# NVlabs/CenterPose

Hardware: AMD Instinct MI355X
Metric: images/sec at 512x512 DLA-34 (backbone + heat-map decode + post-process + PnP) (higher is better)
Workload: dtype f32 via split-f16 (f16x3) MFMA, f32 accumulate

## Files before the change

centerpose_amd/csrc/pw16.hip:

```cpp
#include "igemm16_common.h"

namespace {

constexpr int DA = 6;
constexpr int DB = 3;

template <int NT>
__global__ __launch_bounds__(256, 2) void pw16_kernel(const ConvParams p, const int tiles_m, const int tiles_n) {
    typedef Frag<32> F;
    typedef F::acc_t acc_t;
    const int lane = threadIdx.x & 63;
    const int wid = __builtin_amdgcn_readfirstlane(threadIdx.x >> 6);
    const int tile = tile_of_block(tiles_m, tiles_n);
    const int tn = tile % tiles_n, tm = tile / tiles_n;
    const int M = p.B * p.Ho * p.Wo;
    float afwd, ainv;
    conv_in_scale(p, &afwd, &ainv);

    const int row = tm * 128 + wid * 32 + (lane & 31), half = lane >> 5;
    const int n0 = p.src_c[0] >> 4, n1 = p.nsrc > 1 ? p.src_c[1] >> 4 : 0, n2 = p.nsrc > 2 ? p.src_c[2] >> 4 : 0;
    const __amdgpu_buffer_rsrc_t r0 = make_rsrc(p.src[0], (unsigned)M * (unsigned)p.src_c[0] * 4u);
    const __amdgpu_buffer_rsrc_t r1 = make_rsrc(p.nsrc > 1 ? p.src[1] : p.src[0], p.nsrc > 1 ? (unsigned)M * (unsigned)p.src_c[1] * 4u : 0u);
    const __amdgpu_buffer_rsrc_t r2 = make_rsrc(p.nsrc > 2 ? p.src[2] : p.src[0], p.nsrc > 2 ? (unsigned)M * (unsigned)p.src_c[2] * 4u : 0u);
    const __amdgpu_buffer_rsrc_t r3 = make_rsrc(p.nsrc > 3 ? p.src[3] : p.src[0], p.nsrc > 3 ? (unsigned)M * (unsigned)p.src_c[3] * 4u : 0u);
    const bool live = row < M;
    const unsigned v0 = live ? (unsigned)(row * p.src_c[0] + half * 8) * 4u : OOB;
    const unsigned v1 = live && p.nsrc > 1 ? (unsigned)(row * p.src_c[1] + half * 8) * 4u : OOB;
    const unsigned v2 = live && p.nsrc > 2 ? (unsigned)(row * p.src_c[2] + half * 8) * 4u : OOB;
    const unsigned v3 = live && p.nsrc > 3 ? (unsigned)(row * p.src_c[3] + half * 8) * 4u : OOB;
    const int G = p.Kpad16 >> 4;

    const unsigned w_bytes = (unsigned)((size_t)p.CoutPad * p.Kpad16 * 2);
    const __amdgpu_buffer_rsrc_t r_wh = make_rsrc(p.w16f_hi, w_bytes), r_wl = make_rsrc(p.w16f_lo, w_bytes);
    unsigned bd_off[NT];
#pragma unroll
    for (int j = 0; j < NT; ++j) bd_off[j] = (unsigned)((((tn * NT + j) * G) * 64 + lane) * 16);

    u32x4 ra[DA][2];
    u32x4 rbh[DB][NT], rbl[DB][NT];
    auto issue_a = [&](int set, int g) {
        if (g >= G) return;
        int kk = g;
        if (kk < n0) {
            ra[set][0] = __builtin_amdgcn_raw_buffer_load_b128(r0, (int)v0, kk * 64, 0);
            ra[set][1] = __builtin_amdgcn_raw_buffer_load_b128(r0, (int)v0, kk * 64 + 16, 0);
            return;
        }
        kk -= n0;
        if (kk < n1) {
            ra[set][0] = __builtin_amdgcn_raw_buffer_load_b128(r1, (int)v1, kk * 64, 0);
            ra[set][1] = __builtin_amdgcn_raw_buffer_load_b128(r1, (int)v1, kk * 64 + 16, 0);
            return;
        }
        kk -= n1;
        if (kk < n2) {
            ra[set][0] = __builtin_amdgcn_raw_buffer_load_b128(r2, (int)v2, kk * 64, 0);
            ra[set][1] = __builtin_amdgcn_raw_buffer_load_b128(r2, (int)v2, kk * 64 + 16, 0);
            return;
        }
        kk -= n2;
        ra[set][0] = __builtin_amdgcn_raw_buffer_load_b128(r3, (int)v3, kk * 64, 0);
        ra[set][1] = __builtin_amdgcn_raw_buffer_load_b128(r3, (int)v3, kk * 64 + 16, 0);
    };
    auto issue_b = [&](int set, int g) {
        if (g >= G) return;
#pragma unroll
        for (int j = 0; j < NT; ++j) {
            rbh[set][j] = __builtin_amdgcn_raw_buffer_load_b128(r_wh, (int)bd_off[j], g * 1024, 0);
            rbl[set][j] = __builtin_amdgcn_raw_buffer_load_b128(r_wl, (int)bd_off[j], g * 1024, 0);
        }
    };

    acc_t acc[1][NT];
#pragma unroll
    for (int j = 0; j < NT; ++j)
#pragma unroll
        for (int r = 0; r < F::NACC; ++r) acc[0][j][r] = 0.f;

#pragma unroll
    for (int u = 0; u < DB; ++u) issue_b(u, u);
#pragma unroll
    for (int u = 0; u < DA; ++u) issue_a(u, u);

    for (int g0 = 0; g0 < G; g0 += DA) {
#pragma unroll
        for (int u = 0; u < DA; ++u) {
            const int g = g0 + u;
            if (g < G) {
                const u32x4 x0 = ra[u][0], x1 = ra[u][1];
                const Split2 s0 = split2(__uint_as_float(x0.x) * afwd, __uint_as_float(x0.y) * afwd);
                const Split2 s1 = split2(__uint_as_float(x0.z) * afwd, __uint_as_float(x0.w) * afwd);
                const Split2 s2 = split2(__uint_as_float(x1.x) * afwd, __uint_as_float(x1.y) * afwd);
                const Split2 s3 = split2(__uint_as_float(x1.z) * afwd, __uint_as_float(x1.w) * afwd);
                const u32x4 hv = {s0.hi, s1.hi, s2.hi, s3.hi}, lv = {s0.lo, s1.lo, s2.lo, s3.lo};
                const h8 ah = *reinterpret_cast<const h8*>(&hv), al = *reinterpret_cast<const h8*>(&lv);
                issue_a(u, g + DA);
                __builtin_amdgcn_sched_barrier(0);
                constexpr int DBm = DB;
                const int sb = u % DBm;
#pragma unroll
                for (int j = 0; j < NT; ++j)
                    acc[0][j] = __builtin_amdgcn_mfma_f32_32x32x16_f16(al, *reinterpret_cast<const h8*>(&rbh[sb][j]), acc[0][j], 0, 0, 0);
#pragma unroll
                for (int j = 0; j < NT; ++j)
                    acc[0][j] = __builtin_amdgcn_mfma_f32_32x32x16_f16(ah, *reinterpret_cast<const h8*>(&rbl[sb][j]), acc[0][j], 0, 0, 0);
#pragma unroll
                for (int j = 0; j < NT; ++j)
                    acc[0][j] = __builtin_amdgcn_mfma_f32_32x32x16_f16(ah, *reinterpret_cast<const h8*>(&rbh[sb][j]), acc[0][j], 0, 0, 0);
                __builtin_amdgcn_sched_barrier(0);
                issue_b(sb, g + DB);
                __builtin_amdgcn_sched_barrier(0);
            }
        }
    }
    igemm_epilogue<32, 1, NT, 4, 1, false>(p, acc, tm, tn, wid, 0, lane, ainv);
}

constexpr int PA = 3;
constexpr int PW_PITCH = 80;
constexpr int PW_PLANE = 32 * PW_PITCH;

template <int NT>
__device__ __forceinline__ void pw16s_pool_epilogue(const ConvParams& p, f32x16 (&acc)[1][NT], const int tn, const int lane, const float ainv,
                                                    const bool live, const int pair_row, const int blk) {
    const int lcol = lane & 31, h = lane >> 5, W = p.Wo;
    const bool relu = p.act == CP_ACT_RELU;
    float amax = 0.f;
    if (live) {
        const size_t base = (size_t)(2 * pair_row) * W + 16 * blk;
        const __amdgpu_buffer_rsrc_t ro = make_rsrc(p.out + base * p.ldo, (unsigned)((W + 16) * p.ldo) * 4u);
        const __amdgpu_buffer_rsrc_t rp = make_rsrc(p.pool_out + ((size_t)pair_row * (W >> 1) + 8 * blk) * p.ldo, (unsigned)(8 * p.ldo) * 4u);
#pragma unroll
        for (int j = 0; j < NT; ++j) {
            const int n = tn * (32 * NT) + j * 32 + lcol;
            const float sc = (p.scale ? p.scale[n] : 1.f) * ainv;
            const float sh = p.shift ? p.shift[n] : 0.f;
            const bool n_ok = n < p.Cout;
            float v[16];
#pragma unroll
            for (int r = 0; r < 16; ++r) v[r] = acc[0][j][r] * sc + sh;
            if (relu) {
#pragma unroll
                for (int r = 0; r < 16; ++r) v[r] = fmaxf(v[r], 0.f);
            }
#pragma unroll
            for (int r = 0; r < 16; ++r) amax = fmaxf(amax, fabsf(v[r]));
            const unsigned vo = n_ok ? (unsigned)(4 * h * p.ldo + n) * 4u : 0x80000000u;
#pragma unroll
            for (int r = 0; r < 16; ++r)
                __builtin_amdgcn_raw_buffer_store_b32(__float_as_uint(v[r]), ro, (int)vo, ((r >> 3) * W + (r & 3) + 8 * ((r >> 2) & 1)) * p.ldo * 4, 0);
            const unsigned vp = n_ok ? (unsigned)(2 * h * p.ldo + n) * 4u : 0x80000000u;
#pragma unroll
            for (int q = 0; q < 4; ++q) {
                const int r = 2 * q;
                const float mx = fmaxf(fmaxf(v[r], v[r + 1]), fmaxf(v[r + 8], v[r + 9]));
                __builtin_amdgcn_raw_buffer_store_b32(__float_as_uint(mx), rp, (int)vp, ((q & 1) + 4 * (q >> 1)) * p.ldo * 4, 0);
            }
        }
    }
    if (p.out_amax) cp_amax_commit(p.out_amax, amax);
}

template <int NT, bool POOL>
__global__ __launch_bounds__(256, NT == 2 ? 3 : 2) void pw16s_kernel(const ConvParams p, const int tiles_m, const int tiles_n) {
    typedef Frag<32> F;
    typedef F::acc_t acc_t;
    __shared__ __attribute__((aligned(16))) unsigned char stage_s[4][2 * PW_PLANE];
    const int lane = threadIdx.x & 63;
    const int wid = __builtin_amdgcn_readfirstlane(threadIdx.x >> 6);
    const int tile = tile_of_block(tiles_m, tiles_n);
    const int tn = tile % tiles_n, tm = tile / tiles_n;
    const int M = p.B * p.Ho * p.Wo;
    float afwd, ainv;
    conv_in_scale(p, &afwd, &ainv);
    unsigned char* st_hi = stage_s[wid];
    unsigned char* st_lo = st_hi + PW_PLANE;

    const int grp = 4 * tm + wid, wblk = POOL ? p.Wo >> 4 : 1;
    const int pair_row = POOL ? grp / wblk : 0, blk = POOL ? grp - pair_row * wblk : 0;
    const bool live = !POOL || pair_row < p.B * (p.Ho >> 1);
    const int c4 = lane & 7, row0 = POOL ? 2 * pair_row * p.Wo + 16 * blk + (lane >> 3) : tm * 128 + wid * 32 + (lane >> 3);
    const int n0 = p.src_c[0] >> 5, n1 = p.nsrc > 1 ? p.src_c[1] >> 5 : 0, n2 = p.nsrc > 2 ? p.src_c[2] >> 5 : 0;
    const __amdgpu_buffer_rsrc_t r0 = make_rsrc(p.src[0], (unsigned)M * (unsigned)p.src_c[0] * 4u);
    const __amdgpu_buffer_rsrc_t r1 = make_rsrc(p.nsrc > 1 ? p.src[1] : p.src[0], p.nsrc > 1 ? (unsigned)M * (unsigned)p.src_c[1] * 4u : 0u);
    const __amdgpu_buffer_rsrc_t r2 = make_rsrc(p.nsrc > 2 ? p.src[2] : p.src[0], p.nsrc > 2 ? (unsigned)M * (unsigned)p.src_c[2] * 4u : 0u);
    const __amdgpu_buffer_rsrc_t r3 = make_rsrc(p.nsrc > 3 ? p.src[3] : p.src[0], p.nsrc > 3 ? (unsigned)M * (unsigned)p.src_c[3] * 4u : 0u);
    const int GC = live ? p.Kpad16 >> 5 : 0;

    const unsigned w_bytes = (unsigned)((size_t)p.CoutPad * p.Kpad16 * 2);
    const __amdgpu_buffer_rsrc_t r_wh = make_rsrc(p.w16f_hi, w_bytes), r_wl = make_rsrc(p.w16f_lo, w_bytes);
    const int G = p.Kpad16 >> 4;
    unsigned bd_off[NT];
#pragma unroll
    for (int j = 0; j < NT; ++j) bd_off[j] = (unsigned)((((tn * NT + j) * G) * 64 + lane) * 16);

    u32x4 ra[PA][4];
    u32x4 rbh[DB][NT], rbl[DB][NT];
    auto load4 = [&](u32x4 (&dst)[4], const __amdgpu_buffer_rsrc_t r, const int cs, const int kk) {
        const unsigned v = (unsigned)row0 * (unsigned)(cs * 4) + (unsigned)(c4 * 16);
#pragma unroll
        for (int i = 0; i < 4; ++i)
            dst[i] = __builtin_amdgcn_raw_buffer_load_b128(r, (int)v, kk * 128 + (POOL ? (i >> 1) * p.Wo + (i & 1) * 8 : i * 8) * cs * 4, 0);
    };
    auto issue_a = [&](int set, int c) {
        if (c >= GC) return;
        int kk = c;
        if (kk < n0) { load4(ra[set], r0, p.src_c[0], kk); return; }
        kk -= n0;
        if (kk < n1) { load4(ra[set], r1, p.src_c[1], kk); return; }
        kk -= n1;
        if (kk < n2) { load4(ra[set], r2, p.src_c[2], kk); return; }
        kk -= n2;
        load4(ra[set], r3, p.src_c[3], kk);
    };
    auto issue_b = [&](int set, int g) {
        if (g >= G) return;
#pragma unroll
        for (int j = 0; j < NT; ++j) {
            rbh[set][j] = __builtin_amdgcn_raw_buffer_load_b128(r_wh, (int)bd_off[j], g * 1024, 0);
            rbl[set][j] = __builtin_amdgcn_raw_buffer_load_b128(r_wl, (int)bd_off[j], g * 1024, 0);
        }
    };

    acc_t acc[1][NT];
#pragma unroll
    for (int j = 0; j < NT; ++j)
#pragma unroll
        for (int r = 0; r < F::NACC; ++r) acc[0][j][r] = 0.f;

#pragma unroll
    for (int u = 0; u < DB; ++u) issue_b(u, u);
#pragma unroll
    for (int u = 0; u < PA; ++u) issue_a(u, u);

    const int wr_off = (lane >> 3) * PW_PITCH + c4 * 8;
    const int rd_off = (lane & 31) * PW_PITCH + (lane >> 5) * 16;
    static_assert((2 * PA) % DB == 0, "the B register set of a K step must be a compile-time index");
    for (int c0 = 0; c0 < GC; c0 += PA) {
#pragma unroll
        for (int u = 0; u < PA; ++u) {
            const int c = c0 + u;
            if (c < GC) {
#pragma unroll
                for (int i = 0; i < 4; ++i) {
                    const u32x4 x = ra[u][i];
                    const Split2 s0 = split2(__uint_as_float(x.x) * afwd, __uint_as_float(x.y) * afwd);
                    const Split2 s1 = split2(__uint_as_float(x.z) * afwd, __uint_as_float(x.w) * afwd);
                    *reinterpret_cast<u32x2*>(st_hi + wr_off + 8 * i * PW_PITCH) = u32x2{s0.hi, s1.hi};
                    *reinterpret_cast<u32x2*>(st_lo + wr_off + 8 * i * PW_PITCH) = u32x2{s0.lo, s1.lo};
                }
                issue_a(u, c + PA);
                __builtin_amdgcn_wave_barrier();
                h8 ah[2], al[2];
#pragma unroll
                for (int h = 0; h < 2; ++h) {
                    ah[h] = *reinterpret_cast<const h8*>(st_hi + rd_off + 32 * h);
                    al[h] = *reinterpret_cast<const h8*>(st_lo + rd_off + 32 * h);
                }
                __builtin_amdgcn_wave_barrier();
#pragma unroll
                for (int h = 0; h < 2; ++h) {
                    const int g = 2 * c + h;
                    const int sb = (2 * u + h) % DB;
                    __builtin_amdgcn_sched_barrier(0);
#pragma unroll
                    for (int j = 0; j < NT; ++j)
                        acc[0][j] = __builtin_amdgcn_mfma_f32_32x32x16_f16(al[h], *reinterpret_cast<const h8*>(&rbh[sb][j]), acc[0][j], 0, 0, 0);
#pragma unroll
                    for (int j = 0; j < NT; ++j)
                        acc[0][j] = __builtin_amdgcn_mfma_f32_32x32x16_f16(ah[h], *reinterpret_cast<const h8*>(&rbl[sb][j]), acc[0][j], 0, 0, 0);
#pragma unroll
                    for (int j = 0; j < NT; ++j)
                        acc[0][j] = __builtin_amdgcn_mfma_f32_32x32x16_f16(ah[h], *reinterpret_cast<const h8*>(&rbh[sb][j]), acc[0][j], 0, 0, 0);
                    __builtin_amdgcn_sched_barrier(0);
                    issue_b(sb, g + DB);
                    __builtin_amdgcn_sched_barrier(0);
                }
            }
        }
    }
    if (POOL) pw16s_pool_epilogue<NT>(p, acc, tn, lane, ainv, live, pair_row, blk);
    else igemm_epilogue<32, 1, NT, 4, 1, false>(p, acc, tm, tn, wid, 0, lane, ainv);
}

template <int NT>
int launch_pw16s(const ConvParams& p, hipStream_t stream) {
    const int M = p.B * p.Ho * p.Wo;
    const int tiles_m = (M + 127) / 128, tiles_n = p.CoutPad / (32 * NT);
    if (p.pool_out) hipLaunchKernelGGL((pw16s_kernel<NT, true>), dim3(tiles_m * tiles_n), dim3(256), 0, stream, p, tiles_m, tiles_n);
    else hipLaunchKernelGGL((pw16s_kernel<NT, false>), dim3(tiles_m * tiles_n), dim3(256), 0, stream, p, tiles_m, tiles_n);
    return hipGetLastError() == hipSuccess ? CP_OK : CP_ERR_LAUNCH;
}

template <int NT>
int launch_pw16(const ConvParams& p, hipStream_t stream) {
    const int M = p.B * p.Ho * p.Wo;
    const int tiles_m = (M + 127) / 128, tiles_n = p.CoutPad / (32 * NT);
    hipLaunchKernelGGL((pw16_kernel<NT>), dim3(tiles_m * tiles_n), dim3(256), 0, stream, p, tiles_m, tiles_n);
    return hipGetLastError() == hipSuccess ? CP_OK : CP_ERR_LAUNCH;
}

}

static_assert(DA % DB == 0, "the B register set of a K step must be a compile-time index");

bool cp_pw16_supported(const ConvParams& p) {
    if (!p.w16f_hi || !p.w16f_lo || p.KH != 1 || p.KW != 1 || p.stride != 1 || p.pad != 0 || p.H != p.Ho || p.W != p.Wo)
        return false;
    if (p.offmask || p.gn_in_a || p.gn_in_d || p.gn_in_mr || p.gn_stats || p.splitk > 1 || p.nsrc < 1 || p.nsrc > 4)
        return false;
    if (p.CoutPad % 64 != 0 || p.Kpad16 != p.Cin || p.Cin % 32 != 0) return false;
    int c = 0;
    const size_t M = (size_t)p.B * p.Ho * p.Wo;
    for (int s = 0; s < p.nsrc; ++s) {
        if (p.src_c[s] % 32 != 0 || M * p.src_c[s] * 4 >= (size_t)0xf0000000u) return false;
        c += p.src_c[s];
    }
    return c == p.Cin && (size_t)p.CoutPad * p.Kpad16 * 2 < (size_t)0x7fffffff && M * p.ldo * 4 < (size_t)0xf0000000u;
}

bool cp_pw16_pool_supported(const ConvParams& p) {
    if (!cp_pw16_supported(p) || (p.dbg & CP_SEL_PW16_FRAG_A)) return false;
    if (p.res || p.gn_stats || p.store != CP_STORE_NHWC || p.coff != 0 || (p.act != CP_ACT_NONE && p.act != CP_ACT_RELU)) return false;
    return p.Ho % 2 == 0 && p.Wo % 16 == 0;
}

int cp_launch_pw16(const ConvParams& p, hipStream_t stream) {
    if (!cp_pw16_supported(p) || (p.pool_out && !cp_pw16_pool_supported(p))) return CP_ERR_INVALID;
    if (!(p.dbg & CP_SEL_PW16_FRAG_A)) return p.CoutPad % 128 == 0 ? launch_pw16s<4>(p, stream) : launch_pw16s<2>(p, stream);
    return p.CoutPad % 128 == 0 ? launch_pw16<4>(p, stream) : launch_pw16<2>(p, stream);
}
```

Measured before the change: 4771.

## Stage pointwise-conv weights through LDS shared across waves in pw16 kernel

New measurement: 4791, median of 6. No clear change (+0.4%).

```diff
diff --git a/centerpose_amd/csrc/pw16.hip b/centerpose_amd/csrc/pw16.hip
--- a/centerpose_amd/csrc/pw16.hip
+++ b/centerpose_amd/csrc/pw16.hip
@@ -283,6 +283,170 @@
     else igemm_epilogue<32, 1, NT, 4, 1, false>(p, acc, tm, tn, wid, 0, lane, ainv);
 }
 
+template <class T>
+__device__ __forceinline__ T pw16w_pick(const bool a, const bool b, const bool c, const T x0, const T x1, const T x2, const T x3) {
+    const T t2 = c ? T(x2) : T(x3), t1 = b ? T(x1) : t2;
+    return a ? T(x0) : t1;
+}
+
+template <int NT, bool POOL>
+__global__ __launch_bounds__(256, NT == 2 ? 3 : 2) void pw16w_kernel(const ConvParams p, const int tiles_m, const int tiles_n) {
+    typedef Frag<32> F;
+    typedef F::acc_t acc_t;
+    constexpr int BLK = 4 * NT * 1024;
+    __shared__ __attribute__((aligned(16))) unsigned char stage_s[4][2 * PW_PLANE];
+    __shared__ __attribute__((aligned(16))) unsigned char wts_s[2][BLK];
+    const int lane = threadIdx.x & 63;
+    const int wid = __builtin_amdgcn_readfirstlane(threadIdx.x >> 6);
+    const int tile = tile_of_block(tiles_m, tiles_n);
+    const int tn = tile % tiles_n, tm = tile / tiles_n;
+    const int M = p.B * p.Ho * p.Wo;
+    float afwd, ainv;
+    conv_in_scale(p, &afwd, &ainv);
+    unsigned char* st_hi = stage_s[wid];
+    unsigned char* st_lo = st_hi + PW_PLANE;
+
+    const int grp = 4 * tm + wid, wblk = POOL ? p.Wo >> 4 : 1;
+    const int pair_row = POOL ? grp / wblk : 0, blk = POOL ? grp - pair_row * wblk : 0;
+    const bool live = !POOL || pair_row < p.B * (p.Ho >> 1);
+    const int c4 = lane & 7, row0 = POOL ? 2 * pair_row * p.Wo + 16 * blk + (lane >> 3) : tm * 128 + wid * 32 + (lane >> 3);
+    auto opaque = [](const float* q) __attribute__((always_inline)) {
+        const unsigned long long v = (unsigned long long)q;
+        const unsigned lo = __builtin_amdgcn_readfirstlane((unsigned)v), hi = __builtin_amdgcn_readfirstlane((unsigned)(v >> 32));
+        return (const float*)(((unsigned long long)hi << 32) | lo);
+    };
+    const float* const q0 = opaque(p.src[0]);
+    const float* const q1 = opaque(p.src[1]);
+    const float* const q2 = opaque(p.src[2]);
+    const float* const q3 = opaque(p.src[3]);
+    const int cs0 = __builtin_amdgcn_readfirstlane(p.src_c[0]), cs1 = __builtin_amdgcn_readfirstlane(p.nsrc > 1 ? p.src_c[1] : 0);
+    const int cs2 = __builtin_amdgcn_readfirstlane(p.nsrc > 2 ? p.src_c[2] : 0), cs3 = __builtin_amdgcn_readfirstlane(p.nsrc > 3 ? p.src_c[3] : 0);
+    const int e0 = cs0 >> 5, e1 = e0 + (cs1 >> 5), e2 = e1 + (cs2 >> 5);
+    const int GC = p.Kpad16 >> 5;
+
+    const unsigned w_bytes = (unsigned)((size_t)p.CoutPad * p.Kpad16 * 2);
+    const void* const w_hi = p.w16f_hi;
+    const void* const w_lo = p.w16f_lo;
+    const void* const w_ptr = (wid & 1) ? w_lo : w_hi;
+    const int G = p.Kpad16 >> 4;
+    unsigned bd_off[NT];
+#pragma unroll
+    for (int j = 0; j < NT; ++j) bd_off[j] = (unsigned)((((tn * NT + j) * G) * 64 + lane) * 16);
+    unsigned char* const w_wr = &wts_s[0][0] + wid * (NT * 1024) + lane * 16;
+    const unsigned char* const w_rd = &wts_s[0][0] + lane * 16;
+
+    u32x4 ra[PA][4];
+    u32x4 rw[NT];
+    u32x4 rb[2][2][NT];
+    h8 ah[2], al[2];
+    auto issue_a = [&](int set, int c) __attribute__((always_inline)) {
+        const bool in0 = c < e0, in1 = c < e1, in2 = c < e2;
+        const float* const q = pw16w_pick(in0, in1, in2, q0, q1, q2, q3);
+        const int cs = pw16w_pick(in0, in1, in2, cs0, cs1, cs2, cs3);
+        const int kk = c - pw16w_pick(in0, in1, in2, 0, e0, e1, e2);
+        const __amdgpu_buffer_rsrc_t r = make_rsrc(q, c < GC && live ? (unsigned)M * (unsigned)cs * 4u : 0u);
+        const unsigned v = (unsigned)row0 * (unsigned)(cs * 4) + (unsigned)(c4 * 16);
+#pragma unroll
+        for (int i = 0; i < 4; ++i)
+            ra[set][i] = __builtin_amdgcn_raw_buffer_load_b128(r, (int)v, kk * 128 + (POOL ? (i >> 1) * p.Wo + (i & 1) * 8 : i * 8) * cs * 4, 0);
+    };
+    auto issue_w = [&](int c) __attribute__((always_inline)) {
+        const __amdgpu_buffer_rsrc_t r = make_rsrc(w_ptr, c < GC ? w_bytes : 0u);
+#pragma unroll
+        for (int j = 0; j < NT; ++j) rw[j] = __builtin_amdgcn_raw_buffer_load_b128(r, (int)bd_off[j], (2 * c + (wid >> 1)) * 1024, 0);
+    };
+    auto write_w = [&](int c) __attribute__((always_inline)) {
+#pragma unroll
+        for (int j = 0; j < NT; ++j) *reinterpret_cast<u32x4*>(w_wr + (c & 1) * BLK + j * 1024) = rw[j];
+    };
+    auto read_b = [&](int c, int h) __attribute__((always_inline)) {
+#pragma unroll
+        for (int j = 0; j < NT; ++j) {
+            rb[h][0][j] = *reinterpret_cast<const u32x4*>(w_rd + (c & 1) * BLK + ((2 * h + 0) * NT + j) * 1024);
+            rb[h][1][j] = *reinterpret_cast<const u32x4*>(w_rd + (c & 1) * BLK + ((2 * h + 1) * NT + j) * 1024);
+        }
+    };
+    const int wr_off = (lane >> 3) * PW_PITCH + c4 * 8;
+    const int rd_off = (lane & 31) * PW_PITCH + (lane >> 5) * 16;
+    auto stage_a = [&](const u32x4 (&src)[4]) {
+#pragma unroll
+        for (int i = 0; i < 4; ++i) {
+            const u32x4 x = src[i];
+            const Split2 s0 = split2(__uint_as_float(x.x) * afwd, __uint_as_float(x.y) * afwd);
+            const Split2 s1 = split2(__uint_as_float(x.z) * afwd, __uint_as_float(x.w) * afwd);
+            *reinterpret_cast<u32x2*>(st_hi + wr_off + 8 * i * PW_PITCH) = u32x2{s0.hi, s1.hi};
+            *reinterpret_cast<u32x2*>(st_lo + wr_off + 8 * i * PW_PITCH) = u32x2{s0.lo, s1.lo};
+        }
+    };
+    auto read_a = [&](int h) __attribute__((always_inline)) {
+        ah[h] = *reinterpret_cast<const h8*>(st_hi + rd_off + 32 * h);
+        al[h] = *reinterpret_cast<const h8*>(st_lo + rd_off + 32 * h);
+    };
+
+    acc_t acc[1][NT];
+#pragma unroll
+    for (int j = 0; j < NT; ++j)
+#pragma unroll
+        for (int r = 0; r < F::NACC; ++r) acc[0][j][r] = 0.f;
+    auto mma = [&](int h) __attribute__((always_inline)) {
+        __builtin_amdgcn_sched_barrier(0);
+#pragma unroll
+        for (int j = 0; j < NT; ++j)
+            acc[0][j] = __builtin_amdgcn_mfma_f32_32x32x16_f16(al[h], *reinterpret_cast<const h8*>(&rb[h][0][j]), acc[0][j], 0, 0, 0);
+#pragma unroll
+        for (int j = 0; j < NT; ++j)
+            acc[0][j] = __builtin_amdgcn_mfma_f32_32x32x16_f16(ah[h], *reinterpret_cast<const h8*>(&rb[h][1][j]), acc[0][j], 0, 0, 0);
+#pragma unroll
+        for (int j = 0; j < NT; ++j)
+            acc[0][j] = __builtin_amdgcn_mfma_f32_32x32x16_f16(ah[h], *reinterpret_cast<const h8*>(&rb[h][0][j]), acc[0][j], 0, 0, 0);
+        __builtin_amdgcn_sched_barrier(0);
+    };
+
+    issue_w(0);
+#pragma unroll
+    for (int u = 0; u < PA; ++u) issue_a(u, u);
+    write_w(0);
+    issue_w(1);
+    stage_a(ra[0]);
+    issue_a(0, PA);
+    __builtin_amdgcn_wave_barrier();
+    read_a(0);
+    __syncthreads();
+    read_b(0, 0);
+
+    for (int c0 = 0; c0 < GC; c0 += PA) {
+#pragma unroll
+        for (int u = 0; u < PA; ++u) {
+            const int c = c0 + u;
+            if (c < GC) {
+                read_b(c, 1);
+                read_a(1);
+                write_w(c + 1);
+                issue_w(c + 2);
+                mma(0);
+                __syncthreads();
+                read_b(c + 1, 0);
+                stage_a(ra[(u + 1) % PA]);
+                issue_a((u + 1) % PA, c + 1 + PA);
+                __builtin_amdgcn_wave_barrier();
+                read_a(0);
+                mma(1);
+            }
+        }
+    }
+    if (POOL) pw16s_pool_epilogue<NT>(p, acc, tn, lane, ainv, live, pair_row, blk);
+    else igemm_epilogue<32, 1, NT, 4, 1, false>(p, acc, tm, tn, wid, 0, lane, ainv);
+}
+
+template <int NT>
+int launch_pw16w(const ConvParams& p, hipStream_t stream) {
+    const int M = p.B * p.Ho * p.Wo;
+    const int tiles_m = (M + 127) / 128, tiles_n = p.CoutPad / (32 * NT);
+    if (p.pool_out) hipLaunchKernelGGL((pw16w_kernel<NT, true>), dim3(tiles_m * tiles_n), dim3(256), 0, stream, p, tiles_m, tiles_n);
+    else hipLaunchKernelGGL((pw16w_kernel<NT, false>), dim3(tiles_m * tiles_n), dim3(256), 0, stream, p, tiles_m, tiles_n);
+    return hipGetLastError() == hipSuccess ? CP_OK : CP_ERR_LAUNCH;
+}
+
 template <int NT>
 int launch_pw16s(const ConvParams& p, hipStream_t stream) {
     const int M = p.B * p.Ho * p.Wo;
@@ -327,6 +491,12 @@
 
 int cp_launch_pw16(const ConvParams& p, hipStream_t stream) {
     if (!cp_pw16_supported(p) || (p.pool_out && !cp_pw16_pool_supported(p))) return CP_ERR_INVALID;
-    if (!(p.dbg & CP_SEL_PW16_FRAG_A)) return p.CoutPad % 128 == 0 ? launch_pw16s<4>(p, stream) : launch_pw16s<2>(p, stream);
+#ifndef PW16_LDS_WEIGHTS
+#define PW16_LDS_WEIGHTS 1
+#endif
+    if (!(p.dbg & CP_SEL_PW16_FRAG_A)) {
+        if (PW16_LDS_WEIGHTS) return p.CoutPad % 128 == 0 ? launch_pw16w<4>(p, stream) : launch_pw16w<2>(p, stream);
+        return p.CoutPad % 128 == 0 ? launch_pw16s<4>(p, stream) : launch_pw16s<2>(p, stream);
+    }
     return p.CoutPad % 128 == 0 ? launch_pw16<4>(p, stream) : launch_pw16<2>(p, stream);
 }
```
